# maxrmorrison/promonet

Measured on AMD Instinct MI355X. Metric: audio samples/sec (22.05 kHz), batch-32 10 s utterances, higher is better.
Workload: dtype bf16; 1 GPU; Generator.forward (prepare_features + HiFi-GAN), batch 32 x 10 s per GPU (861 frames, 220416 samples each), random-init weights, bf16 MFMA operands, fp32 accumulate and activations; model=hifigan, batch_per_gpu=32, frames=861, devices=1, parallelism=batch-sharded x1

## Files before the change

include/promonet_hip.h:

```cpp
#ifndef PROMONET_HIP_H
#define PROMONET_HIP_H

#include <stddef.h>
#include <stdint.h>

#ifdef __cplusplus
extern "C" {
#endif

#define PM_OK 0
#define PM_EINVAL (-1)
#define PM_ESTATE (-2)
#define PM_EHIP (-3)
#define PM_ENOMEM (-4)
#define PM_ETIMEOUT (-5)

#define PM_F32 0
#define PM_F16 1
#define PM_BF16 2
#define PM_F16X3 3
#define PM_F16A2 4
#define PM_F16UX 5

#define PM_MAX_STAGES 8
// ... 92 lines not shown
                                      int embedding_channels,
                                      int speaker_channels, void* stream);

size_t pm_op_workspace_bytes(int c_in, int c_out, int k);
int pm_block_iteration_cl(int dtype, const float* x_cl, float* out_cl,
                          const float* w1, const float* b1, const float* w2,
                          const float* b2, int batch, int length,
                          int channels, int kernel_size, int dilation,
                          int mode, float scale, void* workspace,
                          size_t workspace_bytes, void* stream);
int pm_block_iteration_ragged_cl(int dtype, const float* x_cl, float* out_cl,
                                 const float* w1, const float* b1,
                                 const float* w2, const float* b2,
                                 const int* lengths, int batch, int length,
                                 int channels, int kernel_size, int dilation,
                                 int mode, float scale, void* workspace,
                                 size_t workspace_bytes, void* stream);
int pm_block_cl(int dtype, const float* x_cl, float* out_cl,
                const float* const* w1, const float* const* b1,
                const float* const* w2, const float* const* b2,
                const int* dilations, int niter, int batch, int length,
                int channels, int kernel_size, int mode, float scale,
                void* workspace, size_t workspace_bytes, void* stream);
int pm_block_act16_cl(int dtype, int act_dtype, const float* x_cl,
                      float* out_cl, void* act16_cl, const float* const* w1,
                      const float* const* b1, const float* const* w2,
                      const float* const* b2, const int* dilations, int niter,
                      int batch, int length, int channels, int kernel_size,
                      int mode, float scale, void* workspace,
                      size_t workspace_bytes, void* stream);
int pm_mrf_cl(int dtype, const float* x_cl, float* out_cl,
              const float* const* w1, const float* const* b1,
              const float* const* w2, const float* const* b2,
              const int* dilations, int niter, int batch, int length,
              int channels, void* workspace, size_t workspace_bytes,
              void* stream);
int pm_input_conv_cl(int dtype, const float* x_cl, float* out_cl,
                     const float* weight, const float* bias,
                     const float* global_features,
                     const float* speaker_weight, const float* speaker_bias,
                     int global_batch, int global_channels, int batch,
                     int length, int c_in, int c_out, void* workspace,
                     size_t workspace_bytes, void* stream);
int pm_conv_transpose_cl(int dtype, const float* x_cl, float* out_cl,
                         const float* w, const float* bias, int batch,
                         int length, int c_in, int c_out, int rate, int lrelu,
                         void* workspace, size_t workspace_bytes,
                         void* stream);
int pm_conv_transpose_ragged_cl(int dtype, const float* x_cl, float* out_cl,
                                const float* w, const float* bias,
                                const int* lengths, int batch, int length,
                                int c_in, int c_out, int rate, int lrelu,
                                void* workspace, size_t workspace_bytes,
                                void* stream);
int pm_conv_transpose_x16_cl(int dtype, const void* x16_cl, float* out_cl,
                             const float* w, const float* bias, int batch,
                             int length, int c_in, int c_out, int rate,
                             void* workspace, size_t workspace_bytes,
                             void* stream);
int pm_out_conv_tanh(const float* x_cl, const float* w, float* out,
                     int batch, int length, int channels, void* stream);
int pm_debug_timeline(void* dev_buffer);
int pm_debug_force(int walk_nseg, int upsample_groups);
int pm_debug_skew(int mode);
int pm_mfma_probe(int dtype, int iterations, const void* operands,
                  float* sink, int workgroups, void* stream);
size_t pm_walk_scratch_bytes(int batch);
int pm_fold_weight_norm(const float* g, const float* v, float* w, int rows,
                        int cols, void* stream);
int pm_to_channels_last(const float* src, float* dst, int batch, int channels,
                        int frames, int c_pad, void* stream);

int pm_grid_sample(const float* seq, const float* grid, float* out, int rows,
                   int n_in, int n_out, int mode, float scale, float offset,
                   float lo, float hi, void* stream);
int pm_stretch_grid(const float* ppg, int ppg_rows, const int* indices,
                    int n_indices, float* selected, float* grid, int frames,
                    int target_frames, void* stream);

#define PM_FARGAN_MIXED 16
typedef struct pm_fargan_s* pm_fargan_t;
int pm_fargan_create(int num_features, int global_channels, int weight_dtype,
                     pm_fargan_t* out);
int pm_fargan_destroy(pm_fargan_t h);
int pm_fargan_load_tensor(pm_fargan_t h, const char* name, const float* dev,
                          const int64_t* shape, int ndim, void* stream);
int pm_fargan_finalize(pm_fargan_t h, void* stream);
// ... 347 lines not shown
```

promonet_amd/_lib.py:

```python
import ctypes
import os
from pathlib import Path

import torch

LIB_PATH = Path(__file__).parent / 'lib' / 'libpromonet_hip.so'

PM_F32, PM_F16, PM_BF16, PM_F16X3, PM_F16A2, PM_F16UX = 0, 1, 2, 3, 4, 5
DTYPES = {'fp32': PM_F32, 'f32': PM_F32, 'f16': PM_F16, 'fp16': PM_F16,
          'bf16': PM_BF16, 'f16x3': PM_F16X3, 'f16a2': PM_F16A2,
          'f16ux': PM_F16UX,
          'mixed': 16}
MAX_STAGES, MAX_RESBLOCKS, MAX_DILATIONS = 8, 4, 4
SPARSE_METHODS = {None: 0, 'percentile': 1, 'constant': 2, 'topk': 3}
DISC_SPEC_R, DISC_SPEC_CMB, DISC_SPEC_DB = range(3)
FDISC_ACTIVATIONS = {'none': 0, 'relu': 1, 'sigmoid': 2}
(ADV_ABS_DIFF, ADV_SQ_ONE_MINUS, ADV_SQ, ADV_HINGE_ONE_MINUS,
 ADV_HINGE_ONE_PLUS) = range(5)
(OPTIM_MAX, OPTIM_MIN, OPTIM_MEAN, OPTIM_NORM, OPTIM_NORM_SQ, OPTIM_NONFINITE,
 OPTIM_FOUND_INF, OPTIM_INV_SCALE, OPTIM_COEF) = range(9)
OPTIM_STATS = 16

c_float_p = ctypes.c_void_p
c_int64_p = ctypes.POINTER(ctypes.c_int64)
# ... 28 lines not shown
    'pm_hifigan_workspace_bytes': (_S, [_P, _I, _I]),
    'pm_hifigan_hopsize': (_I, [_P]),
    'pm_hifigan_features_cl_channels': (_I, [_P]),
    'pm_hifigan_forward': (_I, [_P, _P, _P, _I, _P, _I, _I, _P, _S, _P]),
    'pm_hifigan_forward_cl': (_I, [_P, _P, _P, _I, _P, _I, _I, _P, _S, _P]),
    'pm_hifigan_forward_ragged': (_I, [_P, _P, _I, _P, _I, _P, _P, _I, _I, _P, _S, _P]),
    'pm_hifigan_context': (_I, [_P, ctypes.POINTER(_I), ctypes.POINTER(_I)]),
    'pm_hifigan_stream': (_I, [_P, _P, _I, _I, _P, _I, _I, _P, _P, _I, _I, _I,
                               _P, _I, _P, _S, _P]),
    'pm_hifigan_stream_workspace_bytes': (_S, [_P, _I, _I]),
    'pm_hifigan_profile_enable': (_I, [_P, _I]),
    'pm_hifigan_profile_only': (_I, [_P, ctypes.c_char_p]),
    'pm_hifigan_profile_collect': (_I, [_P]),
    'pm_hifigan_profile_reset': (_I, [_P]),
    'pm_hifigan_profile_report': (ctypes.c_char_p, [_P]),
    'pm_prepare_features': (_I, [_P] * 8 + [_I] * 9 + [_F] * 6 + [_P]),
    'pm_prepare_global_features': (_I, [_P] * 5 + [_I, _I, _I, _P]),
    'pm_prepare_global_features_linear': (_I, [_P] * 6 + [_I, _I, _I, _P]),
    'pm_op_workspace_bytes': (_S, [_I, _I, _I]),
    'pm_block_iteration_cl': (_I, [_I] + [_P] * 6 + [_I] * 6 + [_F, _P, _S, _P]),
    'pm_block_iteration_ragged_cl': (
        _I, [_I] + [_P] * 7 + [_I] * 6 + [_F, _P, _S, _P]),
    'pm_block_cl': (_I, [_I, _P, _P] + [_P] * 5 + [_I] * 6 + [_F, _P, _S, _P]),
    'pm_block_act16_cl': (
        _I, [_I, _I, _P, _P, _P] + [_P] * 5 + [_I] * 6 + [_F, _P, _S, _P]),
    'pm_mrf_cl': (_I, [_I, _P, _P] + [_P] * 5 + [_I] * 4 + [_P, _S, _P]),
    'pm_input_conv_cl': (_I, [_I] + [_P] * 7 + [_I] * 6 + [_P, _S, _P]),
    'pm_conv_transpose_cl': (_I, [_I] + [_P] * 4 + [_I] * 6 + [_P, _S, _P]),
    'pm_conv_transpose_ragged_cl': (
        _I, [_I] + [_P] * 5 + [_I] * 6 + [_P, _S, _P]),
    'pm_conv_transpose_x16_cl': (_I, [_I] + [_P] * 4 + [_I] * 5 + [_P, _S, _P]),
    'pm_out_conv_tanh': (_I, [_P, _P, _P, _I, _I, _I, _P]),
    'pm_debug_timeline': (_I, [_P]),
    'pm_debug_force': (_I, [_I, _I]),
    'pm_debug_skew': (_I, [_I]),
    'pm_mfma_probe': (_I, [_I, _I, _P, _P, _I, _P]),
    'pm_walk_scratch_bytes': (_S, [_I]),
    'pm_fold_weight_norm': (_I, [_P, _P, _P, _I, _I, _P]),
    'pm_to_channels_last': (_I, [_P, _P, _I, _I, _I, _I, _P]),
    'pm_grid_sample': (_I, [_P, _P, _P, _I, _I, _I, _I, _F, _F, _F, _F, _P]),
    'pm_stretch_grid': (_I, [_P, _I, _P, _I, _P, _P, _I, _I, _P]),
    'pm_fargan_create': (_I, [_I, _I, _I, ctypes.POINTER(_P)]),
    'pm_fargan_destroy': (_I, [_P]),
    'pm_fargan_load_tensor': (_I, [_P, ctypes.c_char_p, _P, c_int64_p, _I, _P]),
    'pm_fargan_finalize': (_I, [_P, _P]),
    'pm_fargan_workspace_bytes': (_S, [_P, _I, _I]),
    'pm_fargan_forward': (_I, [_P, _P, _I, _P, _I, _P, _I, _P, _I, _I, _P, _S, _P]),
    'pm_fargan_forward_ragged': (_I, [_P, _P, _I, _P, _I, _P, _I, _P, _P, _I, _I, _P, _S, _P]),
    'pm_fargan_forward_stateful': (_I, [_P, _P, _I, _P, _I, _P, _I, _P, _P, _P, _P, _I, _I, _P, _S, _P]),
    'pm_fargan_set_mode': (_I, [_P, _I]),
    'pm_fargan_check': (_I, [_P, _I, _I, _P, _P]),
    'pm_stft_scratch_bytes': (_S, [_I, _I]),
    'pm_stft_magnitude': (_I, [_P, _P, _I, _I, _P, _S, _P]),
    'pm_stft_magnitude_dft': (_I, [_P, _P, _I, _I, _P, _S, _P]),
    'pm_stft_mel_scratch_bytes': (_S, [_I]),
    'pm_stft_mel_prepare': (_I, [_P, _I, _P, _S, _P]),
    'pm_stft_mel': (_I, [_P, _P, _P, _I, _I, _I, _I, _F, _P]),
    'pm_stft_set_frames_per_group': (_I, [_I]),
# ... 157 lines not shown
```

promonet_amd/csrc/pm_api.hip:

```cpp
#include <hip/hip_runtime.h>

#include <algorithm>
#include <cstdarg>
#include <cstdio>
#include <cstring>
#include <map>
#include <mutex>
#include <string>
#include <vector>

#include "pm_host.h"
#include "pm_launch.h"
#include "pm_misc.h"

#define PM_VERSION 100

static thread_local char g_error[512] = "";

int pm_fail(int code, const char* fmt, ...) {
    va_list ap;
    va_start(ap, fmt);
    vsnprintf(g_error, sizeof(g_error), fmt, ap);
    va_end(ap);
    return code;
// ... 1066 lines not shown
    void* stream) {
    if (!lengths) return pm_fail(PM_EINVAL, "null argument");
    return block_iteration_cl_impl(dtype, x, out, w1, b1, w2, b2, lengths, B,
                                   L, C, K, d, mode, scale, ws, ws_bytes,
                                   stream);
}

extern "C" int pm_debug_timeline(void* dev_buffer) {
#ifdef PM_TUNING
    g_timeline = (unsigned long long*)dev_buffer;
    return PM_OK;
#else
    (void)dev_buffer;
    return pm_fail(PM_ESTATE, "pm_debug_timeline needs a -DPM_TUNING build "
                              "(make TUNING=1)");
#endif
}

static int block_cl_impl(
    int dtype, const float* x, float* out, const float* const* w1,
    const float* const* b1, const float* const* w2, const float* const* b2,
    const int* dilations, int niter, int B, int L, int C, int K, int mode,
    float scale, void* ws, size_t ws_bytes, void* stream, void* act16,
    int act_dtype) {
    if (!x || !out || !w1 || !b1 || !w2 || !b2 || !dilations || !ws)
        return pm_fail(PM_EINVAL, "null argument");
    const int Cp = pm_pad32(C);
    if (Cp > 256)
        return pm_fail(PM_EINVAL, "channels %d unsupported (<= 256)", C);
    if ((K != 3 && K != 7 && K != 11) || niter < 1 || niter > 3)
        return pm_fail(PM_EINVAL,
                       "kernel %d / %d iterations unsupported", K, niter);
    const size_t per = iteration_layout(C, C, K, nullptr).total;
    if (ws_bytes < 3 * per)
        return pm_fail(PM_ENOMEM, "workspace too small");
    hipStream_t s = (hipStream_t)stream;
    PmStage d = stage_desc(Cp, x, out, B, L, mode, scale, 1, niter);
    d.blk[0].K = K;
    for (int n = 0; n < niter; ++n) {
        const int rc = pack_iteration(dtype, C, K, w1[n], b1[n], w2[n], b2[n],
                                      (char*)ws + n * per, s, &d.blk[0].w1[n],
                                      &d.blk[0].w2[n]);
        if (rc) return rc;
        d.blk[0].dil[n] = dilations[n];
    }
    if (ws_bytes > 3 * per) {
        d.scratch = (char*)ws + 3 * per;
        d.scratch_bytes = ws_bytes - 3 * per;
    }
    if (act16) { d.act16 = act16; d.act16_type = act_dtype; }
    PmPlan plan;
    PM_HIP_TRY(plan_stage(dtype, d, 1, &plan));
    if (plan.block[0].kernel == PM_PAIRS)
        return pm_fail(PM_EINVAL, "no whole-Block kernel for this shape");
    PM_HIP_TRY(launch_block3(dtype, plan.block[0], d, 0, s));
    if (act16 && !plan.block[0].act16)
        return pm_fail(PM_ESTATE,
                       "the launch did not take the skewed walk: `out` "
                       "holds the fp32 result, the 16-bit operand copy was not "
                       "written");
    return PM_OK;
}

extern "C" int pm_block_cl(
    int dtype, const float* x, float* out, const float* const* w1,
    const float* const* b1, const float* const* w2, const float* const* b2,
    const int* dilations, int niter, int B, int L, int C, int K, int mode,
    float scale, void* ws, size_t ws_bytes, void* stream) {
    return block_cl_impl(dtype, x, out, w1, b1, w2, b2, dilations, niter, B, L,
                         C, K, mode, scale, ws, ws_bytes, stream, nullptr, 0);
}

extern "C" int pm_block_act16_cl(
    int dtype, int act_dtype, const float* x, float* out, void* act16,
    const float* const* w1, const float* const* b1, const float* const* w2,
    const float* const* b2, const int* dilations, int niter, int B, int L,
    int C, int K, int mode, float scale, void* ws, size_t ws_bytes,
    void* stream) {
    if (!act16) return pm_fail(PM_EINVAL, "null argument");
    if (act_dtype != PM_F16 && act_dtype != PM_BF16)
        return pm_fail(PM_EINVAL, "act_dtype must be PM_F16 or PM_BF16");
    return block_cl_impl(dtype, x, out, w1, b1, w2, b2, dilations, niter, B, L,
                         C, K, mode, scale, ws, ws_bytes, stream, act16,
                         act_dtype);
}

extern "C" int pm_mrf_cl(
    int dtype, const float* x, float* out, const float* const* w1,
    const float* const* b1, const float* const* w2, const float* const* b2,
    const int* dilations, int niter, int B, int L, int C, void* ws,
    size_t ws_bytes, void* stream) {
    if (!x || !out || !w1 || !b1 || !w2 || !b2 || !dilations || !ws)
        return pm_fail(PM_EINVAL, "null argument");
// ... 170 lines not shown
    const uint4* src = (const uint4*)operands;
    if (dtype == PM_F16)
        hipLaunchKernelGGL(pm_mfma_probe_kernel<1>, dim3(workgroups), dim3(256),
                           0, s, src, sink, iterations);
    else if (dtype == PM_BF16)
        hipLaunchKernelGGL(pm_mfma_probe_kernel<2>, dim3(workgroups), dim3(256),
                           0, s, src, sink, iterations);
    else
        return pm_fail(PM_EINVAL,
                       "probe operand type must be PM_F16 or PM_BF16");
    PM_HIP_TRY(hipGetLastError());
    return PM_OK;
}

extern "C" int pm_debug_skew(int mode) {
    if (!debug_hooks_enabled())
        return pm_fail(PM_ESTATE, "debug hooks are disabled "
                       "(start the process with PROMONET_HIP_DEBUG=1)");
    if (mode < -1 || mode > 1) return pm_fail(PM_EINVAL, "mode is -1, 0 or 1");
    pm_force().skew = mode;
    return PM_OK;
}

extern "C" size_t pm_walk_scratch_bytes(int B) {
    return B < 1 ? 0 : walk_scratch_bytes(B);
}

extern "C" int pm_fold_weight_norm(
    const float* g, const float* v, float* w, int rows, int cols,
    void* stream) {
    if (!g || !v || !w || rows < 1 || cols < 1)
        return pm_fail(PM_EINVAL, "bad argument");
    hipLaunchKernelGGL(pm_fold_kernel, dim3(rows), dim3(256), 0,
                       (hipStream_t)stream, g, v, w, cols);
    PM_HIP_TRY(hipGetLastError());
    return PM_OK;
}

extern "C" int pm_to_channels_last(
    const float* src, float* dst, int B, int C, int T, int c_pad,
    void* stream) {
    if (!src || !dst || c_pad % 32) return pm_fail(PM_EINVAL, "bad argument");
    dim3 grid((T + 31) / 32, c_pad / 32, B);
    hipLaunchKernelGGL(pm_to_channels_last_kernel, grid, dim3(256), 0,
                       (hipStream_t)stream, src, dst, C, T, c_pad);
    PM_HIP_TRY(hipGetLastError());
// ... 41 lines not shown
```

promonet_amd/csrc/pm_conv.h:

```cpp
#pragma once
#include <type_traits>

#include "pm_common.h"


template <class ET, int CH, int NT, int XR_MAX>
struct ChunkStager {
    static constexpr int Q = CH / 4;
    static constexpr int MAXIT = (XR_MAX * Q + NT - 1) / NT;
    static constexpr int S = CH * ET::ESZ + 16;
    float4 r[MAXIT];

    __device__ __forceinline__ void load(
        const float* __restrict__ xb, int cstride, int c0, int t_first,
        int XR, int L, int tid) {
        const int lo = max(t_first, 0);
        const int hi = min(L, t_first + XR);
        const __amdgpu_buffer_rsrc_t rsrc = __builtin_amdgcn_make_buffer_rsrc(
            const_cast<float*>(xb) + (size_t)lo * cstride, 0,
            max(hi - lo, 0) * cstride * 4, 0x00020000);
#pragma unroll
        for (int it = 0; it < MAXIT; ++it) {
            const int idx = tid + it * NT;
            const int row = idx / Q, q = idx % Q;
// ... 447 lines not shown
        for (int k = 0; k < CP / R::CPI; ++k) {
            const float4 v = *reinterpret_cast<const float4*>(
                ebuf + R::at(R::CPI * k + h, q));
            pm_u4 r;
            r.x = __float_as_uint(v.x + bias.x);
            r.y = __float_as_uint(v.y + bias.y);
            r.z = __float_as_uint(v.z + bias.z);
            r.w = __float_as_uint(v.w + bias.w);
            __builtin_amdgcn_raw_buffer_store_b128(
                r, orsrc, voff + (unsigned)(k * R::CPI * M * 4), 0,
                PM_ROWS_AUX);
        }
    }
}

#ifndef PM_OUT_ROWS
#define PM_OUT_ROWS 7
#endif
#ifndef PM_OUT_ROWS_AUX
#define PM_OUT_ROWS_AUX 2
#endif
#ifndef PM_OUT_ROWS_K11
#define PM_OUT_ROWS_K11 0
#endif
template <int MTW, int NTW, int NB, bool ZADD, bool A16>
__device__ __forceinline__ void pm_store_out_rows(
    const floatx16 (&acc)[MTW][NTW], char* ebuf, __amdgpu_buffer_rsrc_t orsrc,
    int C, int m0, int n0, int mode, float scale, int lane,
    __amdgpu_buffer_rsrc_t arsrc, bool a16, bool a16f) {
    typedef RowStores<MTW, 32> R;
    constexpr int KI = 32 / R::CPI;
    const int ln = lane & 31, lh = lane >> 5;
    const int q = lane % R::LPR, h = lane / R::LPR;
    const int q8 = lane % (R::LPR / 2), h8 = lane / (R::LPR / 2);
    const unsigned voff0 = (unsigned)(((n0 + h) * C + m0 + 4 * q) * 4);
    const unsigned voff8 = (unsigned)(((n0 + h8) * C + m0 + 8 * q8) * 4);
    const float s = mode == 0 ? 1.f : scale;
    const bool wide = A16 && a16;
#pragma unroll
    for (int p0 = 0; p0 < NTW; p0 += NB) {
        pm_u4 old[NB][KI] = {};
        if (mode == 2) {
#pragma unroll
            for (int i = 0; i < NB; ++i) {
                if (p0 + i >= NTW) break;
                const unsigned col = (unsigned)((p0 + i) * 32 * C * 4);
// ... 1307 lines not shown
    int nseg;
    int wg_scratch;
    char* scratch;
};

template <class ET, int C, int K, int WM, int WN, int NTW>
struct SkewGeom {
    static constexpr int NC = WN * NTW * 32;
    static constexpr int H2 = (K - 1) / 2;
    static constexpr int AL = 4 * H2;
    static constexpr int S = C * ET::ESZ + 16;
    static constexpr int RA = AL + 32 + NC;
    static constexpr int RT = NC + 2 * H2;
    static constexpr int MTW = (C / 32) / WM;
    static constexpr int NW = WM * WN;
    static constexpr int TB = MTW * 4096;
    static constexpr int CA = 32 + 4 * H2;
    static constexpr int OFF_AC = 2 * 2 * WM * TB;
    static constexpr int OFF_TC = OFF_AC + 3 * CA * S;
    static constexpr int SCRATCH = (OFF_TC + 3 * 2 * H2 * S + 255) & ~255;
    static constexpr int SMEM = (RA + RT) * S;
};

template <class ET, int C, int K, int WM, int WN, int NTW>
__global__ __launch_bounds__(WM * WN * 64) void conv_block3_skew_kernel(
    Block3SkewArgs p) {
    typedef SkewGeom<ET, C, K, WM, WN, NTW> GE;
    typedef typename ET::afrag_t frag_t;
    constexpr int CH = C < 64 ? C : 64;
    constexpr int NCH = C / CH;
    constexpr int KC = CH / 16;
    constexpr int MTW = GE::MTW;
    constexpr int NC = GE::NC;
    constexpr int NT = WM * WN * 64;
    constexpr int H2 = GE::H2;
    constexpr int AL = GE::AL;
    constexpr int S = GE::S;
    constexpr int QS = S / 16;
    constexpr int G = pm_skew_prefetch_depth<ET>(KC);
    constexpr int W_CHUNK = K * KC * 64;
    constexpr int W_BIAS = NCH * W_CHUNK;
    constexpr int W_MT_STRIDE = W_BIAS + 64;
    constexpr int AUX = 16;
    constexpr int PM_SKEW_BD = ET::SPLIT ? 2 : 0;
    static_assert(NTW >= 2, "the trunk shift needs two tiles per wave");


    extern __shared__ __attribute__((aligned(16))) char smem[];
    char* abuf = smem;
// ... 55 lines not shown
    constexpr int TIN = (2 * H2 * QS + NT - 1) / NT;
    constexpr int SIT = (32 * Q + NT - 1) / NT;
    constexpr int PRE = CIN > SIT ? CIN : SIT;
    auto rows_request = [&](int tid, auto& r, int rows, unsigned soff,
                            unsigned dead) {
        constexpr int N = sizeof(r) / sizeof(r[0]);
#pragma unroll
        for (int it = 0; it < N; ++it) {
            const int i = tid + it * NT;
            r[it] = __builtin_amdgcn_raw_buffer_load_b128(
                srsrc, (i < rows * QS ? soff + (unsigned)i * 16 : 0x40000000u) + dead,
                0, AUX);
        }
    };
    auto rows_in = [&](int tid, char* dst, const auto& r, int rows) {
        constexpr int N = sizeof(r) / sizeof(r[0]);
#pragma unroll
        for (int it = 0; it < N; ++it) {
            const int i = tid + it * NT;
            if (i < rows * QS)
                reinterpret_cast<pm_u4*>(dst)[i] = r[it];
        }
    };

#ifdef PM_TUNING
    unsigned long long ph[10] = {};
    unsigned long long last = __builtin_amdgcn_s_memtime();
#define PM_SKEW_MARK(k)                                                       \
    do {                                                                      \
        const unsigned long long now = __builtin_amdgcn_s_memtime();          \
        ph[k] += now - last; last = now;                                      \
    } while (0)
#else
#define PM_SKEW_MARK(k) ((void)0)
#endif
    auto strip_request = [&](int tid, pm_u4 (&r)[PRE], int c_first) {
        const int lo = max(c_first, 0);
        const __amdgpu_buffer_rsrc_t rsrc = __builtin_amdgcn_make_buffer_rsrc(
            const_cast<float*>(xb) + (size_t)lo * C, 0,
            max(min(L, c_first + 32) - lo, 0) * C * 4, 0x00020000);
#pragma unroll
        for (int it = 0; it < SIT; ++it) {
            const int idx = tid + it * NT;
            r[it] = __builtin_amdgcn_raw_buffer_load_b128(
                rsrc, (unsigned)(((c_first - lo) * C + idx * 4) * 4), 0, 0);
        }
// ... 23 lines not shown
                for (int mt = 0; mt < MTW; ++mt)
#pragma unroll
                    for (int nt = 0; nt < NTW; ++nt) trunk[mt][nt] = acc[mt][nt];
            } else {
                const unsigned voff0 = (unsigned)(
                    ((c0 - x_lo + wn * NTW * 32 + ln) * C + m_first + 4 * lh) * 4);
#pragma unroll
                for (int mt = 0; mt < MTW; ++mt)
#pragma unroll
                    for (int nt = 0; nt < NTW; ++nt) {
                        const unsigned voff =
                            voff0 + (unsigned)((mt * 32 + nt * 32 * C) * 4);
#pragma unroll
                        for (int g4 = 0; g4 < 4; ++g4) {
                            const pm_u4 v = __builtin_amdgcn_raw_buffer_load_b128(
                                xrsrc, voff + g4 * 32, 0, 0);
                            trunk[mt][nt][4 * g4 + 0] = __uint_as_float(v.x);
                            trunk[mt][nt][4 * g4 + 1] = __uint_as_float(v.y);
                            trunk[mt][nt][4 * g4 + 2] = __uint_as_float(v.z);
                            trunk[mt][nt][4 * g4 + 3] = __uint_as_float(v.w);
                        }
                    }
            }
            const int d0 = karg->a.dil[0];
            pm_u4 cin[CIN] = {};
            if (d0 > 1) rows_request(tid, cin, H2 * (d0 - 1), GE::OFF_AC, dead);
#pragma unroll
            for (int mt = 0; mt < MTW; ++mt)
#pragma unroll
                for (int nt = 0; nt < NTW; ++nt) {
                    const int col = (wn * NTW + nt) * 32 + ln;
                    store_tile_lrelu_impl<ET, false>(
                        abuf + (AL + col) * S, m_first + mt * 32, trunk[mt][nt],
                        false, lh);
                }
#pragma unroll
            for (int it = 0; it < SIT; ++it) {
                const int idx = tid + it * NT;
                const int r = idx / Q, q = idx % Q;
                if (idx < 32 * Q)
                    ET::store4_at(abuf + (AL + NC + r) * S, q * 4,
                                  pm_lrelu4(make_float4(
                                   __uint_as_float(pre[it].x),
                                   __uint_as_float(pre[it].y),
                                   __uint_as_float(pre[it].z),
                                   __uint_as_float(pre[it].w))));
            }
            if (d0 > 1)
                rows_in(tid, abuf + (AL + H2 - H2 * d0) * S, cin, H2 * (d0 - 1));
        }
        __builtin_amdgcn_s_waitcnt(0x0F70);
        pm_block_sync();
        PM_SKEW_MARK(0);

#pragma unroll 1
        for (int it = 0; it < niter; ++it) {
            const int d = karg->a.dil[it];
            const int o = c0 - 32 * it;
            const bool more = it + 1 < niter;

            bias_start<ET, MTW, NTW>(acc, bf);
            pm_u4 tcin[TIN];
            {
                const int t1 = fresh_tid();
                rows_request(t1, tcin, 2 * H2, GE::OFF_TC + it * 2 * H2 * S, dead);
                const frag_t* w1 = stream_of(karg->a.w1[it], t1);
                const frag_t* w2 = stream_of(karg->a.w2[it], t1);
                const int col_off = col_offset(t1);
#pragma unroll 1
                for (int c = 0; c < NCH; ++c)
                    mma_taps<ET, K, KC, MTW, NTW, G, S, NoHook, PM_SKEW_BD>(
                        acc, abuf + (AL + H2 - H2 * d) * S + col_off + c * CH * ET::ESZ,
                        d * S, w1 + (size_t)c * W_CHUNK, W_MT_STRIDE, afirst,
                        c + 1 < NCH ? w1 + (size_t)(c + 1) * W_CHUNK : w2);
            }
            PM_SKEW_MARK(1);
            const int tid = fresh_tid();
            const int ln = tid & 31, lh = (tid >> 5) & 1;
            load_bias_frags<ET, MTW>(
                bf, stream_of(karg->a.w2[it], tid) + W_BIAS, W_MT_STRIDE);
            {
                const int rows = (it ? 32 : 0) + H2 * (d - 1);
                rows_out(tid, abuf + (AL + NC + H2 - H2 * d) * S, rows,
                         GE::OFF_AC + it * GE::CA * S);
            }
#pragma unroll
            for (int mt = 0; mt < MTW; ++mt)
#pragma unroll
                for (int nt = 0; nt < NTW; ++nt) {
                    const int col_first = (wn * NTW + nt) * 32;
                    store_tile_lrelu<ET>(
                        tbuf + (2 * H2 + col_first + ln) * S, m_first + mt * 32,
                        acc[mt][nt], o + H2 + col_first, L, ln, lh);
                    if (!more) {
                        const int cn = c0 + NC;
                        const __amdgpu_buffer_rsrc_t nrsrc =
                            __builtin_amdgcn_make_buffer_rsrc(
                                const_cast<float*>(xb) + (size_t)cn * C, 0,
                                (cn - skew < e0 ? max(min(L, cn + NC) - cn, 0) : 0) *
                                    C * 4, 0x00020000);
                        const unsigned voff = (unsigned)(
                            ((col_first + ln) * C + m_first + mt * 32 + 4 * lh) * 4);
#pragma unroll
                        for (int g4 = 0; g4 < 4; ++g4) {
                            const pm_u4 v = __builtin_amdgcn_raw_buffer_load_b128(
                                nrsrc, voff + g4 * 32, 0, 0);
                            acc[mt][nt][4 * g4 + 0] = __uint_as_float(v.x);
                            acc[mt][nt][4 * g4 + 1] = __uint_as_float(v.y);
                            acc[mt][nt][4 * g4 + 2] = __uint_as_float(v.z);
                            acc[mt][nt][4 * g4 + 3] = __uint_as_float(v.w);
                        }
                    }
                }
            rows_in(tid, tbuf, tcin, 2 * H2);
            bias_add<ET, MTW, NTW>(trunk, bf);
            PM_SKEW_MARK(2);
            pm_block_sync();
            PM_SKEW_MARK(3);
            {
                const int t2 = fresh_tid();
                if (more)
                    rows_request(t2, pre, 32 + H2 * (karg->a.dil[it + 1] - 1),
                                 GE::OFF_AC + (it + 1) * GE::CA * S, dead);
                else if (c0 + NC - skew < e0)
                    strip_request(t2, pre, c0 + 2 * NC);
                const frag_t* w2 = stream_of(karg->a.w2[it], t2);
                const frag_t* w1n =
                    stream_of(karg->a.w1[more ? it + 1 : it], t2);
                const int col_off = col_offset(t2);
#pragma unroll 1
                for (int c = 0; c < NCH; ++c)
                    mma_taps<ET, K, KC, MTW, NTW, G, S, NoHook, PM_SKEW_BD>(
                        trunk, tbuf + col_off + c * CH * ET::ESZ, S,
                        w2 + (size_t)c * W_CHUNK, W_MT_STRIDE, afirst,
                        c + 1 < NCH ? w2 + (size_t)(c + 1) * W_CHUNK
                                    : (more ? w1n : nullptr));
            }
            PM_SKEW_MARK(4);
            const int te = fresh_tid();
            const int ln2 = te & 31, lh2 = (te >> 5) & 1;
            const unsigned lane_slot = (unsigned)((te & 63) * 16);
            if (more)
                load_bias_frags<ET, MTW>(
                    bf, stream_of(karg->a.w1[it + 1], te) + W_BIAS, W_MT_STRIDE);
            rows_out(te, tbuf + NC * S, 2 * H2, GE::OFF_TC + it * 2 * H2 * S);
            if (more) {
                pm_block_sync();
                if (wn + 1 < WN) {
                    char* slot = tbuf +
                        (2 * H2 + (wn + 1) * NTW * 32 + (te & 63)) * S +
                        m_first * ET::ESZ;
#pragma unroll
                    for (int mt = 0; mt < MTW; ++mt)
#pragma unroll
                        for (int g4 = 0; g4 < 4; ++g4)
                            *reinterpret_cast<float4*>(
                                slot + mt * 32 * ET::ESZ + g4 * 16) =
                                acc_quad(trunk[mt][NTW - 1], g4);
                } else {
                    const unsigned xo =
                        (unsigned)(((par * 2 + it) * WM + wm) * GE::TB) +
                        lane_slot;
#pragma unroll
                    for (int mt = 0; mt < MTW; ++mt)
#pragma unroll
                        for (int g4 = 0; g4 < 4; ++g4) {
                            const floatx16& v = trunk[mt][NTW - 1];
                            const pm_u4 u = {__float_as_uint(v[4 * g4 + 0]),
                                             __float_as_uint(v[4 * g4 + 1]),
                                             __float_as_uint(v[4 * g4 + 2]),
                                             __float_as_uint(v[4 * g4 + 3])};
                            __builtin_amdgcn_raw_buffer_store_b128(
                                u, srsrc, xo + mt * 4096 + g4 * 1024, 0, 0);
                        }
                }
                const int dn = karg->a.dil[it + 1];
#pragma unroll
                for (int mt = 0; mt < MTW; ++mt)
#pragma unroll
                    for (int nt = 0; nt < NTW; ++nt) {
                        const int col_first = (wn * NTW + nt) * 32;
                        store_tile_lrelu<ET>(
                            abuf + (AL + 32 + col_first + ln2) * S,
                            m_first + mt * 32, trunk[mt][nt], o + col_first, L,
                            ln2, lh2);
                    }
#pragma unroll
                for (int mt = 0; mt < MTW; ++mt)
#pragma unroll
                    for (int nt = NTW - 1; nt > 0; --nt)
                        trunk[mt][nt] = trunk[mt][nt - 1];
                rows_in(te, abuf + (AL + H2 - H2 * dn) * S, pre,
                        32 + H2 * (dn - 1));
                PM_SKEW_MARK(5);
                pm_block_sync();
                PM_SKEW_MARK(7);
                if (wn > 0) {
                    const char* slot = tbuf +
                        (2 * H2 + wn * NTW * 32 + (te & 63)) * S +
                        m_first * ET::ESZ;
#pragma unroll
                    for (int mt = 0; mt < MTW; ++mt)
#pragma unroll
                        for (int g4 = 0; g4 < 4; ++g4) {
                            const float4 v = *reinterpret_cast<const float4*>(
                                slot + mt * 32 * ET::ESZ + g4 * 16);
                            trunk[mt][0][4 * g4 + 0] = v.x;
                            trunk[mt][0][4 * g4 + 1] = v.y;
                            trunk[mt][0][4 * g4 + 2] = v.z;
                            trunk[mt][0][4 * g4 + 3] = v.w;
                        }
                } else {
                    const unsigned xi =
                        (unsigned)((((par ^ 1) * 2 + it) * WM + wm) * GE::TB) +
                        dead;
#pragma unroll
// ... 606 lines not shown
```

promonet_amd/csrc/pm_launch.h:

```cpp
#pragma once
#include <algorithm>
#include <cstdlib>
#include <cstring>
#include <map>
#include <mutex>
#include <utility>

#include "pm_conv.h"
#include "pm_host.h"

struct PmForce { int walk_nseg = 0; int upsample_groups = 0; int skew = 0; };
#define PM_SKEW_WG_SCRATCH (256 << 10)
inline PmForce& pm_force() { static thread_local PmForce f; return f; }

inline bool pm_narrow_allowed() {
#ifdef PM_TUNING
    static const bool allowed = !getenv("PM_NO_NARROW");
    return allowed;
#else
    return true;
#endif
}

inline int pm_fusion_level() {
#ifdef PM_TUNING
    static const int level = [] {
        const char* e = getenv("PM_FUSION");
        return (e && !strcmp(e, "pair")) ? 0 : (e && !strcmp(e, "block")) ? 1 : 2;
    }();
    return level;
#else
    return 2;
#endif
}
// ... 58 lines not shown
template <> struct Block3Cfg<ElemF16, 128, 7>  { enum { WM = 4, WN = 2, NTW = 4 }; };
template <> struct Block3Cfg<ElemF16, 128, 11> { enum { WM = 4, WN = 2, NTW = 4 }; };
template <> struct Block3Cfg<ElemF16, 256, 3>  { enum { WM = 8, WN = 1, NTW = 4 }; };
template <> struct Block3Cfg<ElemF16, 256, 7>  { enum { WM = 8, WN = 1, NTW = 4 }; };
template <int C, int K> struct Block3Cfg<ElemBF16, C, K> : Block3Cfg<ElemF16, C, K> {};
template <> struct Block3Cfg<ElemF32, 32, 3>   { enum { WM = 1, WN = 8, NTW = 2 }; };
template <> struct Block3Cfg<ElemF32, 32, 7>   { enum { WM = 1, WN = 8, NTW = 2 }; };
template <> struct Block3Cfg<ElemF32, 32, 11>  { enum { WM = 1, WN = 8, NTW = 2 }; };
template <> struct Block3Cfg<ElemF32, 64, 3>   { enum { WM = 2, WN = 4, NTW = 2 }; };
template <> struct Block3Cfg<ElemF32, 64, 7>   { enum { WM = 2, WN = 4, NTW = 2 }; };
template <> struct Block3Cfg<ElemF32, 64, 11>  { enum { WM = 2, WN = 4, NTW = 2 }; };
template <int C, int K> struct Block3Cfg<ElemF16X3, C, K> : Block3Cfg<ElemF32, C, K> {};
template <int C, int K> struct Block3Cfg<ElemF16A2, C, K> : Block3Cfg<ElemF32, C, K> {};

template <class ET, int C, int K> struct Block3CfgNarrow : Block3Cfg<ET, C, K> {};
template <> struct Block3CfgNarrow<ElemF16, 32, 11> { enum { WM = 1, WN = 4, NTW = 3 }; };
template <> struct Block3CfgNarrow<ElemF16, 64, 7>  { enum { WM = 2, WN = 2, NTW = 4 }; };
template <> struct Block3CfgNarrow<ElemF16, 64, 11> { enum { WM = 2, WN = 2, NTW = 4 }; };
template <> struct Block3CfgNarrow<ElemF16, 128, 3> { enum { WM = 4, WN = 1, NTW = 4 }; };
template <int C, int K> struct Block3CfgNarrow<ElemBF16, C, K> : Block3CfgNarrow<ElemF16, C, K> {};

template <class ET, int C>
constexpr bool pm_skew_4byte() { return ET::ESZ == 4 && (C == 32 || C == 64); }

template <class ET, int C, int K, class G> struct Block3Kernels {
    static constexpr int NW = G::WM * G::WN;
    static constexpr bool SKEW = G::WM != 0 && NW == 8 && G::NTW >= 2 &&
                                 (ET::ESZ == 2 || pm_skew_4byte<ET, C>());
    static constexpr bool WALK = G::WM != 0 && NW == 8 && ET::ESZ == 2 &&
                                 !(C == 128 && K == 11) && !(C == 256 && K == 7);
    static constexpr bool TILED = G::WM != 0 && !(C == 128 && K >= 7) && C != 256;
};
template <class ET, class G> struct MrfKernels {
    static constexpr int NW = G::WM * G::WN;
    static constexpr bool ANY = G::WM != 0 && Block3Cfg<ET, 32, 3>::WM != 0 &&
                                Block3Cfg<ET, 32, 7>::WM != 0;
    static constexpr bool SKEW = ANY && ET::ESZ == 4 && NW == 8 && G::NTW >= 2;
    static constexpr bool WALK = ANY && ET::ESZ == 2 && NW == 8;
};

struct PmBlock {
    int K;
    const void* w1[PM_MAX_DILATIONS];
    const void* w2[PM_MAX_DILATIONS];
    int dil[PM_MAX_DILATIONS];
};
// ... 2 lines not shown
    const float* x;
    float* out;
    int B, L;
    const int* lengths;
    int len_scale;
    int mode;
    float scale;
    char* scratch;
    size_t scratch_bytes;
    void* act16;
    int act16_type;
    int nblocks, niter;
    PmBlock blk[PM_MAX_RESBLOCKS];
    PM_TIMELINE_FIELD
};

enum PmKernel { PM_PAIRS, PM_SKEW, PM_WALK, PM_TILED };
struct PmLaunch {
    PmKernel kernel = PM_PAIRS;
    bool narrow = false;
    int halo = 0;
    int nseg = 0;
    bool act16 = false;
};
struct PmPlan {
    bool mrf = false;
    PmLaunch block[PM_MAX_RESBLOCKS];
};

inline int pm_halo(int K, int niter, const int* dil) {
    int halo = 0;
    for (int i = 0; i < niter; ++i) halo += (dil[i] + 1) * ((K - 1) / 2);
    return halo;
}
inline bool pm_skew_dilations(int K, int niter, const int* dil) {
    for (int i = 0; i < niter; ++i)
        if (dil[i] < 1 || dil[i] > 5 || ((K - 1) / 2) * (dil[i] + 1) > 30)
            return false;
    return true;
}
inline int pm_walk_segments(int B) {
    if (pm_force().walk_nseg) return pm_force().walk_nseg;
    const int cus = pm_device_cus();
    return cus > 0 ? std::max(1, cus / B) : 0;
}
inline bool pm_take_narrow(int nc_wide, int nc_narrow, int halo, int B, int L) {
// ... 26 lines not shown
    typedef Block3Kernels<ET, C, K, G> KS;
    if constexpr (G::WM == 0) {
        return false;
    } else {
    constexpr int NC = G::WN * G::NTW * 32;
    const int* dil = s.blk[j].dil;
    l->halo = pm_halo(K, s.niter, dil);
    if (NC - 2 * l->halo < 32) return false;
    const PmForce& f = pm_force();
    const int nseg = pm_walk_segments(s.B);
    if constexpr (KS::SKEW) {
        typedef SkewGeom<ET, C, K, G::WM, G::WN, G::NTW> GE;
        static_assert(GE::SCRATCH <= PM_SKEW_WG_SCRATCH, "scratch bound");
        constexpr bool WINS = ((C == 128 || C == 64) && K >= 7) ||
                              pm_skew_4byte<ET, C>();
        if (GE::SMEM <= PM_LDS_BYTES && s.scratch && nseg > 0 &&
            (f.skew > 0 || (f.skew == 0 && WINS)) &&
            pm_skew_dilations(K, s.niter, dil) &&
            (f.walk_nseg || (s.L / NC) / nseg >= 4) &&
            (size_t)s.B * nseg * GE::SCRATCH <= s.scratch_bytes) {
            l->kernel = PM_SKEW;
            l->nseg = nseg;
            l->act16 = s.act16 && j == s.nblocks - 1;
            return true;
        }
    }
    if constexpr (KS::WALK) {
        const int smem = block3_walk_smem_bytes<ET, C, K, G::WM, G::WN, G::NTW>() +
                         block3_carry_bytes<ET, C>(l->halo);
        if (smem <= PM_LDS_BYTES && nseg > 0 &&
            (f.walk_nseg || (s.L / (NC - l->halo)) / nseg >= 6)) {
            l->kernel = PM_WALK;
            l->nseg = nseg;
            return true;
        }
    }
    if constexpr (KS::TILED) {
        l->kernel = PM_TILED;
        return true;
    }
    return false;
    }
}

template <class ET, int C, int K>
static PmLaunch plan_block_ck(const PmStage& s, int j) {
// ... 169 lines not shown
        a.dil[n] = s.blk[j].dil[n];
    }
    a.B = s.B; a.L = s.L; a.mode = j == 0 ? s.mode : 2; a.scale = s.scale;
    a.halo = halo; a.TL = NC - 2 * halo; a.ntiles = (s.L + a.TL - 1) / a.TL;
    a.lengths = s.lengths; a.len_scale = s.len_scale;
#ifdef PM_TUNING
    a.timeline = s.timeline;
#endif
    return a;
}

template <class ET, int C, int K, class G>
static hipError_t launch_block3_cfg(const PmLaunch& l, const PmStage& s, int j,
                                    hipStream_t stream) {
    typedef Block3Kernels<ET, C, K, G> KS;
    constexpr int WM = G::WM, WN = G::WN, NTW = G::NTW, NT = WM * WN * 64;
    Block3Args a = block3_args(s, j, WN * NTW * 32, l.halo);
    if constexpr (KS::SKEW) if (l.kernel == PM_SKEW) {
        typedef SkewGeom<ET, C, K, WM, WN, NTW> GE;
        if (l.act16) { a.act16 = s.act16; a.act16_type = s.act16_type; }
        Block3SkewArgs p;
        p.a = a; p.nseg = l.nseg; p.wg_scratch = GE::SCRATCH;
        p.scratch = s.scratch;
        return launch_with_lds(conv_block3_skew_kernel<ET, C, K, WM, WN, NTW>,
                               a.B * l.nseg, NT, GE::SMEM, stream, p);
    }
    if constexpr (KS::WALK) if (l.kernel == PM_WALK) {
        Block3WalkArgs p;
        p.a = a; p.nseg = l.nseg;
        return launch_with_lds(
            conv_block3_walk_kernel<ET, C, K, WM, WN, NTW>, a.B * l.nseg, NT,
            block3_walk_smem_bytes<ET, C, K, WM, WN, NTW>() +
                block3_carry_bytes<ET, C>(a.halo),
            stream, p);
    }
    if constexpr (KS::TILED) if (l.kernel == PM_TILED)
        return launch_with_lds(conv_block3_kernel<ET, C, K, WM, WN, NTW>,
                               a.ntiles * a.B, NT,
                               block3_smem_bytes<ET, C, K, WM, WN, NTW>(), stream, a);
    return hipErrorInvalidValue;
}

template <class ET, int C, int K>
static hipError_t launch_block3_ck(const PmLaunch& l, const PmStage& s, int j,
                                   hipStream_t stream) {
    return l.narrow
// ... 196 lines not shown
```

Baseline: 417.6 million samples/s.

## Keep skew-kernel halo carries in registers instead of global scratch

Adds a register-carry variant of the skewed residual-block kernel for 2-byte element types with C=64/128, K>=7 and three iterations starting at dilation 1. Halo rows that were written to and reloaded from per-workgroup global scratch are now held in rotating register arrays across segment steps. This removes scratch round trips and their request latency from the inner loop, at the cost of more VGPR pressure that may reduce occupancy or cause spills. It also adds a ragged block entry point and a debug switch to disable the carry path.

```diff
diff --git a/include/promonet_hip.h b/include/promonet_hip.h
--- a/include/promonet_hip.h
+++ b/include/promonet_hip.h
@@ -138,6 +138,13 @@
                 const int* dilations, int niter, int batch, int length,
                 int channels, int kernel_size, int mode, float scale,
                 void* workspace, size_t workspace_bytes, void* stream);
+int pm_block_ragged_cl(int dtype, const float* x_cl, float* out_cl,
+                       const float* const* w1, const float* const* b1,
+                       const float* const* w2, const float* const* b2,
+                       const int* dilations, const int* lengths, int niter,
+                       int batch, int length, int channels, int kernel_size,
+                       int mode, float scale, void* workspace,
+                       size_t workspace_bytes, void* stream);
 int pm_block_act16_cl(int dtype, int act_dtype, const float* x_cl,
                       float* out_cl, void* act16_cl, const float* const* w1,
                       const float* const* b1, const float* const* w2,
@@ -179,6 +186,7 @@
 int pm_debug_timeline(void* dev_buffer);
 int pm_debug_force(int walk_nseg, int upsample_groups);
 int pm_debug_skew(int mode);
+int pm_debug_skew_carries(int mode);
 int pm_mfma_probe(int dtype, int iterations, const void* operands,
                   float* sink, int workgroups, void* stream);
 size_t pm_walk_scratch_bytes(int batch);
diff --git a/promonet_amd/_lib.py b/promonet_amd/_lib.py
--- a/promonet_amd/_lib.py
+++ b/promonet_amd/_lib.py
@@ -74,6 +74,8 @@
     'pm_block_iteration_ragged_cl': (
         _I, [_I] + [_P] * 7 + [_I] * 6 + [_F, _P, _S, _P]),
     'pm_block_cl': (_I, [_I, _P, _P] + [_P] * 5 + [_I] * 6 + [_F, _P, _S, _P]),
+    'pm_block_ragged_cl': (
+        _I, [_I, _P, _P] + [_P] * 6 + [_I] * 6 + [_F, _P, _S, _P]),
     'pm_block_act16_cl': (
         _I, [_I, _I, _P, _P, _P] + [_P] * 5 + [_I] * 6 + [_F, _P, _S, _P]),
     'pm_mrf_cl': (_I, [_I, _P, _P] + [_P] * 5 + [_I] * 4 + [_P, _S, _P]),
@@ -86,6 +88,7 @@
     'pm_debug_timeline': (_I, [_P]),
     'pm_debug_force': (_I, [_I, _I]),
     'pm_debug_skew': (_I, [_I]),
+    'pm_debug_skew_carries': (_I, [_I]),
     'pm_mfma_probe': (_I, [_I, _I, _P, _P, _I, _P]),
     'pm_walk_scratch_bytes': (_S, [_I]),
     'pm_fold_weight_norm': (_I, [_P, _P, _P, _I, _I, _P]),
diff --git a/promonet_amd/csrc/pm_api.hip b/promonet_amd/csrc/pm_api.hip
--- a/promonet_amd/csrc/pm_api.hip
+++ b/promonet_amd/csrc/pm_api.hip
@@ -1112,7 +1112,7 @@
     const float* const* b1, const float* const* w2, const float* const* b2,
     const int* dilations, int niter, int B, int L, int C, int K, int mode,
     float scale, void* ws, size_t ws_bytes, void* stream, void* act16,
-    int act_dtype) {
+    int act_dtype, const int* lengths = nullptr) {
     if (!x || !out || !w1 || !b1 || !w2 || !b2 || !dilations || !ws)
         return pm_fail(PM_EINVAL, "null argument");
     const int Cp = pm_pad32(C);
@@ -1126,6 +1126,7 @@
         return pm_fail(PM_ENOMEM, "workspace too small");
     hipStream_t s = (hipStream_t)stream;
     PmStage d = stage_desc(Cp, x, out, B, L, mode, scale, 1, niter);
+    d.lengths = lengths; d.len_scale = 1;
     d.blk[0].K = K;
     for (int n = 0; n < niter; ++n) {
         const int rc = pack_iteration(dtype, C, K, w1[n], b1[n], w2[n], b2[n],
@@ -1159,6 +1160,17 @@
     float scale, void* ws, size_t ws_bytes, void* stream) {
     return block_cl_impl(dtype, x, out, w1, b1, w2, b2, dilations, niter, B, L,
                          C, K, mode, scale, ws, ws_bytes, stream, nullptr, 0);
+}
+
+extern "C" int pm_block_ragged_cl(
+    int dtype, const float* x, float* out, const float* const* w1,
+    const float* const* b1, const float* const* w2, const float* const* b2,
+    const int* dilations, const int* lengths, int niter, int B, int L, int C,
+    int K, int mode, float scale, void* ws, size_t ws_bytes, void* stream) {
+    if (!lengths) return pm_fail(PM_EINVAL, "null argument");
+    return block_cl_impl(dtype, x, out, w1, b1, w2, b2, dilations, niter, B, L,
+                         C, K, mode, scale, ws, ws_bytes, stream, nullptr, 0,
+                         lengths);
 }
 
 extern "C" int pm_block_act16_cl(
@@ -1375,6 +1387,15 @@
     return PM_OK;
 }
 
+extern "C" int pm_debug_skew_carries(int mode) {
+    if (!debug_hooks_enabled())
+        return pm_fail(PM_ESTATE, "debug hooks are disabled "
+                       "(start the process with PROMONET_HIP_DEBUG=1)");
+    if (mode < -1 || mode > 0) return pm_fail(PM_EINVAL, "mode is -1 or 0");
+    pm_force().skew_carries = mode;
+    return PM_OK;
+}
+
 extern "C" size_t pm_walk_scratch_bytes(int B) {
     return B < 1 ? 0 : walk_scratch_bytes(B);
 }
diff --git a/promonet_amd/csrc/pm_conv.h b/promonet_amd/csrc/pm_conv.h
--- a/promonet_amd/csrc/pm_conv.h
+++ b/promonet_amd/csrc/pm_conv.h
@@ -493,6 +493,9 @@
 #endif
 #ifndef PM_OUT_ROWS_K11
 #define PM_OUT_ROWS_K11 0
+#endif
+#ifndef PM_SKEW_CARRY_REGS
+#define PM_SKEW_CARRY_REGS 1
 #endif
 template <int MTW, int NTW, int NB, bool ZADD, bool A16>
 __device__ __forceinline__ void pm_store_out_rows(
@@ -1846,9 +1849,29 @@
     static constexpr int SMEM = (RA + RT) * S;
 };
 
-template <class ET, int C, int K, int WM, int WN, int NTW>
+struct ElemBF16Regs {};
+struct ElemF16Regs {};
+template <class ET> struct SkewCarryRegs { typedef void type; };
+template <> struct SkewCarryRegs<ElemBF16> { typedef ElemBF16Regs type; };
+template <> struct SkewCarryRegs<ElemF16> { typedef ElemF16Regs type; };
+template <class EF> struct SkewForm {
+    typedef EF elem;
+    static constexpr bool CARRY = false;
+};
+template <> struct SkewForm<ElemBF16Regs> {
+    typedef ElemBF16 elem;
+    static constexpr bool CARRY = true;
+};
+template <> struct SkewForm<ElemF16Regs> {
+    typedef ElemF16 elem;
+    static constexpr bool CARRY = true;
+};
+
+template <class EF, int C, int K, int WM, int WN, int NTW>
 __global__ __launch_bounds__(WM * WN * 64) void conv_block3_skew_kernel(
     Block3SkewArgs p) {
+    typedef typename SkewForm<EF>::elem ET;
+    constexpr bool CARRY = SkewForm<EF>::CARRY;
     typedef SkewGeom<ET, C, K, WM, WN, NTW> GE;
     typedef typename ET::afrag_t frag_t;
     constexpr int CH = C < 64 ? C : 64;
@@ -1950,6 +1973,17 @@
                 reinterpret_cast<pm_u4*>(dst)[i] = r[it];
         }
     };
+    auto rows_keep = [&](int tid, auto& r, const char* src, int rows) {
+        constexpr int N = sizeof(r) / sizeof(r[0]);
+#pragma unroll
+        for (int it = 0; it < N; ++it) {
+            const int i = tid + it * NT;
+            if (i < rows * QS)
+                r[it] = reinterpret_cast<const pm_u4*>(src)[i];
+        }
+    };
+    pm_u4 acar[CARRY ? 2 : 1][CIN] = {};
+    pm_u4 tcar[CARRY ? 3 : 1][TIN] = {};
 
 #ifdef PM_TUNING
     unsigned long long ph[10] = {};
@@ -2019,7 +2053,7 @@
                         }
                     }
             }
-            const int d0 = karg->a.dil[0];
+            const int d0 = CARRY ? 1 : karg->a.dil[0];
             pm_u4 cin[CIN] = {};
             if (d0 > 1) rows_request(tid, cin, H2 * (d0 - 1), GE::OFF_AC, dead);
 #pragma unroll
@@ -2060,7 +2094,9 @@
             pm_u4 tcin[TIN];
             {
                 const int t1 = fresh_tid();
-                rows_request(t1, tcin, 2 * H2, GE::OFF_TC + it * 2 * H2 * S, dead);
+                if constexpr (!CARRY)
+                    rows_request(t1, tcin, 2 * H2, GE::OFF_TC + it * 2 * H2 * S,
+                                 dead);
                 const frag_t* w1 = stream_of(karg->a.w1[it], t1);
                 const frag_t* w2 = stream_of(karg->a.w2[it], t1);
                 const int col_off = col_offset(t1);
@@ -2078,8 +2114,15 @@
                 bf, stream_of(karg->a.w2[it], tid) + W_BIAS, W_MT_STRIDE);
             {
                 const int rows = (it ? 32 : 0) + H2 * (d - 1);
-                rows_out(tid, abuf + (AL + NC + H2 - H2 * d) * S, rows,
-                         GE::OFF_AC + it * GE::CA * S);
+                if constexpr (!CARRY) {
+                    rows_out(tid, abuf + (AL + NC + H2 - H2 * d) * S, rows,
+                             GE::OFF_AC + it * GE::CA * S);
+                } else if (it) {
+#pragma unroll
+                    for (int q = 0; q < CIN; ++q) acar[0][q] = acar[1][q];
+                    rows_keep(tid, acar[1], abuf + (AL + NC + H2 - H2 * d) * S,
+                              rows);
+                }
             }
 #pragma unroll
             for (int mt = 0; mt < MTW; ++mt)
@@ -2109,17 +2152,20 @@
                         }
                     }
                 }
-            rows_in(tid, tbuf, tcin, 2 * H2);
+            if constexpr (CARRY) rows_in(tid, tbuf, tcar[0], 2 * H2);
+            else rows_in(tid, tbuf, tcin, 2 * H2);
             bias_add<ET, MTW, NTW>(trunk, bf);
             PM_SKEW_MARK(2);
             pm_block_sync();
             PM_SKEW_MARK(3);
             {
                 const int t2 = fresh_tid();
-                if (more)
-                    rows_request(t2, pre, 32 + H2 * (karg->a.dil[it + 1] - 1),
-                                 GE::OFF_AC + (it + 1) * GE::CA * S, dead);
-                else if (c0 + NC - skew < e0)
+                if (more) {
+                    if constexpr (!CARRY)
+                        rows_request(t2, pre,
+                                     32 + H2 * (karg->a.dil[it + 1] - 1),
+                                     GE::OFF_AC + (it + 1) * GE::CA * S, dead);
+                } else if (c0 + NC - skew < e0)
                     strip_request(t2, pre, c0 + 2 * NC);
                 const frag_t* w2 = stream_of(karg->a.w2[it], t2);
                 const frag_t* w1n =
@@ -2140,7 +2186,16 @@
             if (more)
                 load_bias_frags<ET, MTW>(
                     bf, stream_of(karg->a.w1[it + 1], te) + W_BIAS, W_MT_STRIDE);
-            rows_out(te, tbuf + NC * S, 2 * H2, GE::OFF_TC + it * 2 * H2 * S);
+            if constexpr (CARRY) {
+#pragma unroll
+                for (int q = 0; q < TIN; ++q) {
+                    tcar[0][q] = tcar[1][q];
+                    tcar[1][q] = tcar[2][q];
+                }
+                rows_keep(te, tcar[2], tbuf + NC * S, 2 * H2);
+            } else
+                rows_out(te, tbuf + NC * S, 2 * H2,
+                         GE::OFF_TC + it * 2 * H2 * S);
             if (more) {
                 pm_block_sync();
                 if (wn + 1 < WN) {
@@ -2187,8 +2242,12 @@
 #pragma unroll
                     for (int nt = NTW - 1; nt > 0; --nt)
                         trunk[mt][nt] = trunk[mt][nt - 1];
-                rows_in(te, abuf + (AL + H2 - H2 * dn) * S, pre,
-                        32 + H2 * (dn - 1));
+                if constexpr (CARRY)
+                    rows_in(te, abuf + (AL + H2 - H2 * dn) * S, acar[0],
+                            32 + H2 * (dn - 1));
+                else
+                    rows_in(te, abuf + (AL + H2 - H2 * dn) * S, pre,
+                            32 + H2 * (dn - 1));
                 PM_SKEW_MARK(5);
                 pm_block_sync();
                 PM_SKEW_MARK(7);
diff --git a/promonet_amd/csrc/pm_launch.h b/promonet_amd/csrc/pm_launch.h
--- a/promonet_amd/csrc/pm_launch.h
+++ b/promonet_amd/csrc/pm_launch.h
@@ -4,12 +4,16 @@
 #include <cstring>
 #include <map>
 #include <mutex>
+#include <type_traits>
 #include <utility>
 
 #include "pm_conv.h"
 #include "pm_host.h"
 
-struct PmForce { int walk_nseg = 0; int upsample_groups = 0; int skew = 0; };
+struct PmForce {
+    int walk_nseg = 0; int upsample_groups = 0; int skew = 0;
+    int skew_carries = 0;
+};
 #define PM_SKEW_WG_SCRATCH (256 << 10)
 inline PmForce& pm_force() { static thread_local PmForce f; return f; }
 
@@ -114,6 +118,12 @@
 
 template <class ET, int C>
 constexpr bool pm_skew_4byte() { return ET::ESZ == 4 && (C == 32 || C == 64); }
+template <class ET, int C, int K>
+constexpr bool pm_skew_carry_regs() {
+    return PM_SKEW_CARRY_REGS && ET::ESZ == 2 && !ET::SPLIT &&
+           !std::is_void<typename SkewCarryRegs<ET>::type>::value &&
+           (C == 128 || C == 64) && K >= 7;
+}
 
 template <class ET, int C, int K, class G> struct Block3Kernels {
     static constexpr int NW = G::WM * G::WN;
@@ -162,6 +172,7 @@
     int halo = 0;
     int nseg = 0;
     bool act16 = false;
+    bool carry_regs = false;
 };
 struct PmPlan {
     bool mrf = false;
@@ -234,6 +245,8 @@
             l->kernel = PM_SKEW;
             l->nseg = nseg;
             l->act16 = s.act16 && j == s.nblocks - 1;
+            l->carry_regs = pm_skew_carry_regs<ET, C, K>() && s.niter == 3 &&
+                            dil[0] == 1 && f.skew_carries >= 0;
             return true;
         }
     }
@@ -449,6 +462,13 @@
         Block3SkewArgs p;
         p.a = a; p.nseg = l.nseg; p.wg_scratch = GE::SCRATCH;
         p.scratch = s.scratch;
+#if PM_SKEW_CARRY_REGS
+        if constexpr (pm_skew_carry_regs<ET, C, K>()) if (l.carry_regs)
+            return launch_with_lds(
+                conv_block3_skew_kernel<typename SkewCarryRegs<ET>::type, C, K,
+                                        WM, WN, NTW>,
+                a.B * l.nseg, NT, GE::SMEM, stream, p);
+#endif
         return launch_with_lds(conv_block3_skew_kernel<ET, C, K, WM, WN, NTW>,
                                a.B * l.nseg, NT, GE::SMEM, stream, p);
     }
```

Result: no change. 420.4 million samples/s (median of 6 runs) (+0.7%).
